# entrpn/learning-jax-sharding

Hardware: AMD Instinct MI355X
Metric: step-time ms + TFLOPS/GPU, case6 sharded attention block at 1/2/4/8 MI355X (higher is better)
Workload: dtype bf16; 1 GPU; model=case6 attention block (M=640, heads=8x64, bf16 compute, f32 params, Adam), global_batch=64, seq_len=256, parallelism=dp1, mode=train, hip_graph=True, graph_segments=1, steps_per_graph=6, warmup_steps_run=67, comm=none, grad_wire=fp32, loss=y.sum(), rules=reference

## Files before the change

learning_jax_sharding_amd/csrc/kernels/gemm.hip:

```cpp
#include "common.h"
#include <stdio.h>
#include <stdlib.h>
#include <type_traits>

namespace {

constexpr int BK = 64;

struct GemmArgs {
  const bf16_t* A;
  const bf16_t* B;
  void* C;
  const void* bias;
  long lda, ldb, ldc;
  long sA, sB, sC, sBias;
  int M, N, K;
  int batch, splitk, kt_per_split;
  float alpha;
  int flags;
  float* psum;
  const void* res;
  long ldr, sR;
  const bf16_t* bptr[4];
  unsigned long long* trace;
};

constexpr int kTraceSlots = 128;

constexpr int kResAdd = 64, kResMask = 128, kResF32 = 256;
constexpr int kSlabs = 512;
constexpr int kMFast = 1024;
constexpr int kBPtrs = 4096;
constexpr int kSlabVst = 8192;

__device__ __forceinline__ void apply_res8(float* v, int flags, const u32x4& rb, const u32x4& rf0,
                                           const u32x4& rf1) {
  float r[8];
  if (flags & kResF32) {
#pragma unroll
    for (int e = 0; e < 4; ++e) { r[e] = __uint_as_float(rf0[e]); r[4 + e] = __uint_as_float(rf1[e]); }
  } else {
#pragma unroll
    for (int e = 0; e < 4; ++e) {
      r[2 * e] = __uint_as_float(rb[e] << 16);
      r[2 * e + 1] = __uint_as_float(rb[e] & 0xffff0000u);
    }
  }
  if (flags & kResAdd) {
#pragma unroll
    for (int e = 0; e < 8; ++e) v[e] = bf2f(f2bf(v[e])) + bf2f(f2bf(r[e]));
  } else if (flags & kResMask) {
#pragma unroll
    for (int e = 0; e < 8; ++e) v[e] = r[e] > 0.f ? v[e] : 0.f;
  }
}

template <int R>
__device__ __forceinline__ int swz_mn(int krow, int c8) {
  int f;
  if constexpr (R >= 128) f = ((krow & 3) | (((krow >> 3) & 1) << 2)) << 2;
  else f = ((((krow >> 1) & 1)) | (((krow >> 3) & 1) << 1)) << 2;
  return c8 ^ f;
}

__device__ __forceinline__ int swz_k(int row, int c16) { return c16 ^ ((row >> 1) & 7); }

template <int R, bool KC>
struct Stage {
  static constexpr int CHUNKS = R * BK * 2 / 16 / 256;
  u32x4 v[CHUNKS];

  __device__ __forceinline__ void load(const bf16_t* __restrict__ base, long ld, int r0, int k0, int R_lim,
                                       int K, int tid) {
#pragma unroll
    for (int i = 0; i < CHUNKS; ++i) {
      int c = tid + 256 * i;
      if constexpr (KC) {
        int row = c >> 3, kc = c & 7;
        int gr = r0 + row, gk = k0 + kc * 8;
        if (gr < R_lim && gk < K)
          v[i] = *reinterpret_cast<const u32x4*>(base + (long)gr * ld + gk);
        else
          v[i] = u32x4{0, 0, 0, 0};
      } else {
        constexpr int CPR = R / 8;
        int krow = c / CPR, mc = c % CPR;
        int gk = k0 + krow, gr = r0 + mc * 8;
        if (gk < K && gr < R_lim)
          v[i] = *reinterpret_cast<const u32x4*>(base + (long)gk * ld + gr);
        else
          v[i] = u32x4{0, 0, 0, 0};
      }
    }
  }

  __device__ __forceinline__ void store(bf16_t* lds, int tid) const {
#pragma unroll
    for (int i = 0; i < CHUNKS; ++i) {
      int c = tid + 256 * i;
      if constexpr (KC) {
        int row = c >> 3, kc = c & 7;
        *reinterpret_cast<u32x4*>(lds + row * BK + swz_k(row, kc) * 8) = v[i];
      } else {
        constexpr int CPR = R / 8;
        int krow = c / CPR, mc = c % CPR;
        *reinterpret_cast<u32x4*>(lds + krow * R + swz_mn<R>(krow, mc * 2) * 4) = v[i];
      }
    }
  }
};

template <int R, bool KC>
__device__ __forceinline__ bf16x8 frag(const bf16_t* lds, int rb, int ks, int lane) {
  if constexpr (KC) {
    int row = rb + (lane & 15);
    int kc = ks * 4 + (lane >> 4);
    u32x4 raw = *reinterpret_cast<const u32x4*>(lds + row * BK + swz_k(row, kc) * 8);
    return __builtin_bit_cast(bf16x8, raw);
  } else {
    int g = lane >> 4, i = lane & 15, q = i >> 2, p = i & 3;
    int kr0 = ks * 32 + 8 * g + q;
    int c8 = (rb >> 2) + p;
    s16x4 lo = lds_read_tr16(lds + kr0 * R + swz_mn<R>(kr0, c8) * 4);
    int kr1 = kr0 + 4;
    s16x4 hi = lds_read_tr16(lds + kr1 * R + swz_mn<R>(kr1, c8) * 4);
    return join_bf16x8(lo, hi);
  }
}

template <int BM, int BN, bool A_KC, bool B_KC, bool OUT_F32>
__global__ __launch_bounds__(256) void gemm_bf16_kernel(GemmArgs p) {
  constexpr int TM = BM / 32, TN = BN / 32;
  constexpr int A_TILE = BM * BK, B_TILE = BN * BK;
  __shared__ __attribute__((aligned(16))) bf16_t smem[2 * (A_TILE + B_TILE)];
#define As(i) (smem + (i) * A_TILE)
#define Bs(i) (smem + 2 * A_TILE + (i) * B_TILE)

  const int tid = threadIdx.x, lane = tid & 63, wave = tid >> 6;
  const int wr = wave >> 1, wc = wave & 1;
  const int ntm = (p.M + BM - 1) / BM, ntn = (p.N + BN - 1) / BN;
  const int tile = xcd_remap(blockIdx.x, gridDim.x);
  const int tm_i = tile / ntn, tn_i = tile % ntn;
  if (tm_i >= ntm) return;
  const int bz = blockIdx.y;
  const int b = bz / p.splitk, split = bz % p.splitk;
  const int m0 = tm_i * BM, n0 = tn_i * BN;

  const bf16_t* Ab = p.A + (long)b * p.sA;
  const bf16_t* Bb = p.B + (long)b * p.sB;

  const int nkt_total = (p.K + BK - 1) / BK;
  const int kt_begin = split * p.kt_per_split;
  const int kt_end = min(nkt_total, kt_begin + p.kt_per_split);

  f32x4 acc[TM][TN];
#pragma unroll
  for (int i = 0; i < TM; ++i)
#pragma unroll
    for (int j = 0; j < TN; ++j) acc[i][j] = f32x4{0.f, 0.f, 0.f, 0.f};

  Stage<BM, A_KC> sa;
  Stage<BN, B_KC> sb;
  if (kt_begin < kt_end) {
    sa.load(Ab, p.lda, m0, kt_begin * BK, p.M, p.K, tid);
    sb.load(Bb, p.ldb, n0, kt_begin * BK, p.N, p.K, tid);
    sa.store(As(0), tid);
    sb.store(Bs(0), tid);
  }
  __syncthreads();

  for (int kt = kt_begin; kt < kt_end; ++kt) {
    const int cur = (kt - kt_begin) & 1;
    const bool more = kt + 1 < kt_end;
    if (more) {
      sa.load(Ab, p.lda, m0, (kt + 1) * BK, p.M, p.K, tid);
      sb.load(Bb, p.ldb, n0, (kt + 1) * BK, p.N, p.K, tid);
    }
#pragma unroll
    for (int ks = 0; ks < BK / 32; ++ks) {
      bf16x8 af[TM], bfr[TN];
#pragma unroll
      for (int i = 0; i < TM; ++i) af[i] = frag<BM, A_KC>(As(cur), wr * (BM / 2) + i * 16, ks, lane);
#pragma unroll
      for (int j = 0; j < TN; ++j) bfr[j] = frag<BN, B_KC>(Bs(cur), wc * (BN / 2) + j * 16, ks, lane);
#pragma unroll
      for (int i = 0; i < TM; ++i)
#pragma unroll
        for (int j = 0; j < TN; ++j) acc[i][j] = mfma16x16x32(af[i], bfr[j], acc[i][j]);
    }
    if (more) {
      sa.store(As(cur ^ 1), tid);
      sb.store(Bs(cur ^ 1), tid);
    }
    __syncthreads();
  }

  const bool relu = p.flags & 1;
  const bool has_bias = (p.flags & 2) && p.splitk == 1;
  const bool bias_f32 = p.flags & 4;
  const bool accumulate = p.flags & 8;
  if constexpr (!OUT_F32) {
    constexpr int LDC = BN + 8;
    bf16_t* ct = smem;
#pragma unroll
    for (int j = 0; j < TN; ++j) {
      const int cl = wc * (BN / 2) + j * 16 + (lane & 15);
      const int col = n0 + cl;
      float bv = 0.f;
      if (has_bias && col < p.N) {
        const long bo = (long)b * p.sBias + col;
        bv = bias_f32 ? reinterpret_cast<const float*>(p.bias)[bo]
                      : bf2f(reinterpret_cast<const bf16_t*>(p.bias)[bo]);
      }
#pragma unroll
      for (int i = 0; i < TM; ++i)
#pragma unroll
        for (int r = 0; r < 4; ++r) {
          float v = acc[i][j][r] * p.alpha + bv;
          if (relu) v = fmaxf(v, 0.f);
          ct[(wr * (BM / 2) + i * 16 + (lane >> 4) * 4 + r) * LDC + cl] = f2bf(v);
        }
    }
    __syncthreads();
    bf16_t* Cb = reinterpret_cast<bf16_t*>(p.C) + (long)b * p.sC;
    constexpr int CPR = BN / 8;
    const bool vec_ok = (p.ldc % 8 == 0) && ((((uintptr_t)Cb) & 15) == 0);
    for (int c = tid; c < BM * CPR; c += 256) {
      const int rl = c / CPR, cc = c % CPR;
      const int row = m0 + rl, col = n0 + cc * 8;
      if (row >= p.M || col >= p.N) continue;
      const bf16_t* src = ct + rl * LDC + cc * 8;
      bf16_t* dst = Cb + (long)row * p.ldc + col;
      if (p.flags & (kResAdd | kResMask)) {
        float v[8];
        u32x4 rb = {0, 0, 0, 0}, rf0 = {0, 0, 0, 0}, rf1 = {0, 0, 0, 0};
        const long ro = (long)b * p.sR + (long)row * p.ldr + col;
#pragma unroll
        for (int e = 0; e < 8; ++e) {
          v[e] = bf2f(src[e]);
          if (col + e < p.N) {
            if (p.flags & kResF32) {
              const float rv = reinterpret_cast<const float*>(p.res)[ro + e];
              if (e < 4) rf0[e] = __float_as_uint(rv); else rf1[e - 4] = __float_as_uint(rv);
            } else {
              const unsigned rv = reinterpret_cast<const bf16_t*>(p.res)[ro + e];
              rb[e >> 1] |= (e & 1) ? (rv << 16) : rv;
            }
          }
        }
        apply_res8(v, p.flags, rb, rf0, rf1);
        if (vec_ok && col + 8 <= p.N)
          *reinterpret_cast<u32x4*>(dst) = u32x4{pack_bf16x2(v[0], v[1]), pack_bf16x2(v[2], v[3]),
                                                 pack_bf16x2(v[4], v[5]), pack_bf16x2(v[6], v[7])};
        else
          for (int e = 0; e < 8 && col + e < p.N; ++e) dst[e] = f2bf(v[e]);
      } else if (vec_ok && col + 8 <= p.N) {
        *reinterpret_cast<u32x4*>(dst) = *reinterpret_cast<const u32x4*>(src);
      } else {
        for (int e = 0; e < 8 && col + e < p.N; ++e) dst[e] = src[e];
      }
    }
    return;
  }
#pragma unroll
  for (int i = 0; i < TM; ++i) {
#pragma unroll
    for (int j = 0; j < TN; ++j) {
      const int col = n0 + wc * (BN / 2) + j * 16 + (lane & 15);
      if (col >= p.N) continue;
      float bv = 0.f;
      if (has_bias) {
        const long bo = (long)b * p.sBias + col;
        bv = bias_f32 ? reinterpret_cast<const float*>(p.bias)[bo]
                      : bf2f(reinterpret_cast<const bf16_t*>(p.bias)[bo]);
      }
#pragma unroll
      for (int r = 0; r < 4; ++r) {
        const int row = m0 + wr * (BM / 2) + i * 16 + (lane >> 4) * 4 + r;
        if (row >= p.M) continue;
        float v = acc[i][j][r] * p.alpha + bv;
        if (relu) v = fmaxf(v, 0.f);
        const long off = (long)b * p.sC + (long)row * p.ldc + col;
        if constexpr (OUT_F32) {
          float* C = reinterpret_cast<float*>(p.C);
          if (p.splitk > 1) atomicAdd(C + off, v);
          else if (accumulate) C[off] += v;
          else C[off] = v;
        } else {
          reinterpret_cast<bf16_t*>(p.C)[off] = f2bf(v);
        }
      }
    }
  }
}

#undef As
#undef Bs


template <int R>
__device__ __forceinline__ int swz_mn16(int krow) {
  if constexpr (R >= 128) return ((krow & 3) | (((krow >> 3) & 1) << 2)) << 1;
  else return ((((krow >> 1) & 1)) | (((krow >> 3) & 1) << 1)) << 1;
}


template <int N>
__device__ __forceinline__ void wait_vm_imm() {
  asm volatile("s_waitcnt vmcnt(%0)" ::"n"(N) : "memory");
}
__device__ __forceinline__ void wait_vm_n(int n) {
  switch (n) {
#define LJS_W(k) case k: wait_vm_imm<k>(); return;
    LJS_W(0) LJS_W(1) LJS_W(2) LJS_W(3) LJS_W(4) LJS_W(5) LJS_W(6) LJS_W(7) LJS_W(8) LJS_W(9) LJS_W(10)
    LJS_W(11) LJS_W(12) LJS_W(13) LJS_W(14) LJS_W(15) LJS_W(16) LJS_W(17) LJS_W(18) LJS_W(19) LJS_W(20)
    LJS_W(21) LJS_W(22) LJS_W(23) LJS_W(24) LJS_W(25) LJS_W(26) LJS_W(27) LJS_W(28) LJS_W(29) LJS_W(30)
    LJS_W(31) LJS_W(32) LJS_W(33) LJS_W(34) LJS_W(35) LJS_W(36) LJS_W(37) LJS_W(38) LJS_W(39) LJS_W(40)
    LJS_W(41) LJS_W(42) LJS_W(43) LJS_W(44) LJS_W(45) LJS_W(46)
#undef LJS_W
    default: wait_vm_imm<47>(); return;
  }
}

template <int R, bool KC, int NW>
struct DmaTile {
  static constexpr int PIECES = R * BK * 2 / 1024;
  static constexpr int PER_WAVE = PIECES / NW;
  static_assert(PIECES % NW == 0, "pieces must split evenly over the waves");
  int voff[PER_WAVE];

  __device__ __forceinline__ void init(long ld, int wave, int lane) {
#pragma unroll
    for (int i = 0; i < PER_WAVE; ++i) {
      const int q = wave + NW * i;
      long e;
      if constexpr (KC) {
        const int row = 8 * q + (lane >> 3), slot = lane & 7;
        e = (long)row * ld + 8 * (slot ^ ((row >> 1) & 7));
      } else {
        constexpr int CPR = R / 8;
        constexpr int KPP = 64 / CPR;
        const int krow = KPP * q + lane / CPR, slot = lane % CPR;
        e = (long)krow * ld + 8 * (slot ^ swz_mn16<R>(krow));
      }
      voff[i] = (int)(e * 2);
    }
  }

  __device__ __forceinline__ void issue(__amdgpu_buffer_rsrc_t rs, bf16_t* lds, int soff, int wave) const {
#pragma unroll
    for (int i = 0; i < PER_WAVE; ++i)
      __builtin_amdgcn_raw_ptr_buffer_load_lds(rs, (LDS_PTR(void))(lds + (wave + NW * i) * 512), 16, voff[i], soff,
                                               0, 0);
  }
};

struct WorkItem {
  int b, m0, n0, kt0, split;
};

__device__ __forceinline__ WorkItem decode_item(const GemmArgs& p, int item, int ntm, int ntn) {
  WorkItem w;
  int tm_i, tn_i, r;
  if (p.flags & kMFast) {
    tm_i = item % ntm;
    r = item / ntm;
    tn_i = r % ntn;
    r /= ntn;
  } else {
    tn_i = item % ntn;
    r = item / ntn;
    tm_i = r % ntm;
    r /= ntm;
  }
  w.b = r % p.batch;
  w.split = r / p.batch;
  w.m0 = tm_i;
  w.n0 = tn_i;
  w.kt0 = w.split * p.kt_per_split;
  return w;
}

constexpr int kSC1 = 16;

template <int BM, int BN, int WM, int WN, int NST, bool A_KC, bool B_KC, bool OUT_F32, int RES = 0>
__device__ __forceinline__ void gemm_dma_body(const GemmArgs& p, const int bid, const int G) {
  constexpr int NW = WM * WN;
  constexpr int TM = BM / WM / 16, TN = BN / WN / 16;
  constexpr int A_TILE = BM * BK, B_TILE = BN * BK, STAGE = A_TILE + B_TILE;
  using TA = DmaTile<BM, A_KC, NW>;
  using TB = DmaTile<BN, B_KC, NW>;
  constexpr int L = TA::PER_WAVE + TB::PER_WAVE;
  constexpr bool SWAP = true;
  static_assert(OUT_F32 || TN % 2 == 0, "column blocks pair up for 16-byte stores");
  constexpr int S_EPI = TM * TN / 2;
  static_assert(L * (NST - 1) + S_EPI + 1 <= 63, "vmcnt immediate range");
  __shared__ __attribute__((aligned(16))) bf16_t smem[NST * STAGE];

  const int tid = threadIdx.x, lane = tid & 63;
  const int wave = __builtin_amdgcn_readfirstlane(tid >> 6);
  const int wr = wave / WN, wc = wave % WN;
  const int ntm = (p.M + BM - 1) / BM, ntn = (p.N + BN - 1) / BN;
  const int items = p.batch * p.splitk * ntm * ntn;
  const int slot = xcd_remap(bid, G);
  const int my_items = slot < items ? (items - slot + G - 1) / G : 0;
  const int nk = p.kt_per_split;
  const int total = my_items * nk;
#ifdef LJS_GEMM_TRACE
  unsigned long long* trc = p.trace ? p.trace + ((long)bid * NW + wave) * kTraceSlots : nullptr;
  int trn = 0;
  auto stamp = [&]() {
    if (trc && trn < kTraceSlots - 1) {
      const unsigned long long t = __builtin_amdgcn_s_memtime();
      if (lane == 0) trc[trn] = t;
    }
    ++trn;
  };
  auto stamp_end = [&]() {
    if (trc) {
      const unsigned long long t = __builtin_amdgcn_s_memtime();
      if (lane == 0) trc[kTraceSlots - 1] = t;
    }
  };
#else
  auto stamp = [&]() {};
  auto stamp_end = [&]() {};
#endif
  stamp();

  constexpr int AES = 2;
  const long a_bytes = AES * (A_KC ? (long)(p.M - 1) * p.lda + p.K : (long)(p.K - 1) * p.lda + p.M);
  const long b_bytes = 2 * (B_KC ? (long)(p.N - 1) * p.ldb + p.K : (long)(p.K - 1) * p.ldb + p.N);
  const long a_kt = A_KC ? (long)BK * AES : (long)BK * p.lda * 2;
  const long b_kt = B_KC ? (long)BK * 2 : (long)BK * p.ldb * 2;

  TA ta;
  TB tb;
  ta.init(p.lda, wave, lane);
  tb.init(p.ldb, wave, lane);

  int is_item = 0, is_kt = 0;
  __amdgpu_buffer_rsrc_t ra, rb;
  int a_off = 0, b_off = 0;
  const int a_step = (int)a_kt, b_step = (int)b_kt;
  auto load_item = [&](int k) {
    const WorkItem w = decode_item(p, slot + G * k, ntm, ntn);
    ra = make_rsrc(reinterpret_cast<const unsigned char*>(p.A) + (long)w.b * p.sA * AES, a_bytes);
    rb = make_rsrc((p.flags & kBPtrs) ? p.bptr[w.b] : p.B + (long)w.b * p.sB, b_bytes);
    a_off = __builtin_amdgcn_readfirstlane(
        (int)((A_KC ? (long)w.m0 * BM * p.lda : (long)w.m0 * BM) * AES + w.kt0 * a_kt));
    b_off = __builtin_amdgcn_readfirstlane(
        (int)((B_KC ? (long)w.n0 * BN * p.ldb : (long)w.n0 * BN) * 2 + w.kt0 * b_kt));
  };
  auto issue_a = [&](int st) { ta.issue(ra, smem + st * STAGE, a_off, wave); };
  auto issue_b = [&](int st) { tb.issue(rb, smem + st * STAGE + A_TILE, b_off, wave); };
  auto issue_next = [&](int st) {
    if (is_kt == 0) load_item(is_item);
    issue_a(st);
    issue_b(st);
    a_off += a_step;
    b_off += b_step;
    if (++is_kt == nk) { is_kt = 0; ++is_item; }
  };
  auto issue_half = [&](int st, bool second) {
    if (!second) {
      if (is_kt == 0) load_item(is_item);
      issue_a(st);
      a_off += a_step;
    } else {
      issue_b(st);
      b_off += b_step;
      if (++is_kt == nk) { is_kt = 0; ++is_item; }
    }
  };

  f32x4 acc[TM][TN];
#pragma unroll
  for (int i = 0; i < TM; ++i)
#pragma unroll
    for (int j = 0; j < TN; ++j) acc[i][j] = f32x4{0.f, 0.f, 0.f, 0.f};

#pragma unroll
  for (int s = 0; s < NST - 1; ++s)
    if (s < total) issue_next(s);

  constexpr bool PLAIN = RES == 3, BSUM = RES == 4, NOALPHA = PLAIN || BSUM;
  constexpr bool HAS_R = RES == 1 || RES == 2;
  const bool relu = !PLAIN && !BSUM && (p.flags & 1);
  const bool has_bias = BSUM || (!PLAIN && (p.flags & 2) && p.splitk == 1);
  const bool bias_f32 = BSUM || (p.flags & 4);
  const bool accumulate = !PLAIN && (p.flags & 8);
  const bool st_sc1 = p.flags & 32;
  const bool psum_on = !OUT_F32 && !PLAIN && p.psum != nullptr;
  float tsum = 0.f;
  const bool slabs = OUT_F32 && (PLAIN || (p.flags & kSlabs));
  const __amdgpu_buffer_rsrc_t rc = make_rsrc(
      p.C, (OUT_F32 ? 4 : 2) *
               ((long)((slabs ? p.splitk * p.batch : p.batch) - 1) * p.sC + (long)(p.M - 1) * p.ldc + p.N));
  bool after_epi = false;

  auto wait_landed = [&](int g) {
    stamp();
    const bool tail = g + NST - 2 >= total;
    if constexpr (NST >= 3) {
      if (tail) asm volatile("s_waitcnt vmcnt(0)" ::: "memory");
      else if (SWAP && after_epi && psum_on)
        asm volatile("s_waitcnt vmcnt(%0)" ::"n"(L * (NST - 2) + S_EPI + 1) : "memory");
      else if (SWAP && after_epi) asm volatile("s_waitcnt vmcnt(%0)" ::"n"(L * (NST - 2) + S_EPI) : "memory");
      else asm volatile("s_waitcnt vmcnt(%0)" ::"n"(L * (NST - 2)) : "memory");
    } else {
      if (SWAP && after_epi && psum_on) asm volatile("s_waitcnt vmcnt(%0)" ::"n"(S_EPI + 1) : "memory");
      else if (SWAP && after_epi) asm volatile("s_waitcnt vmcnt(%0)" ::"n"(S_EPI) : "memory");
      else asm volatile("s_waitcnt vmcnt(0)" ::: "memory");
    }
    after_epi = false;
    stamp();
    asm volatile("s_waitcnt lgkmcnt(0)" ::: "memory");
    __builtin_amdgcn_s_barrier();
    stamp();
  };
  bf16x8 ka[TM], kb[TN], la[TM], lb[TN];
  auto read_frags = [&](int g, int ks, bf16x8* af, bf16x8* bfr) {
    const bf16_t* As_ = smem + (g % NST) * STAGE;
    const bf16_t* Bs_ = As_ + A_TILE;
#pragma unroll
    for (int ii = 0; ii < TM; ++ii) af[ii] = frag<BM, A_KC>(As_, wr * (BM / WM) + ii * 16, ks, lane);
#pragma unroll
    for (int j = 0; j < TN; ++j) bfr[j] = frag<BN, B_KC>(Bs_, wc * (BN / WN) + j * 16, ks, lane);
  };
  auto mfmas = [&](const bf16x8* af, const bf16x8* bfr) {
#pragma unroll
    for (int ii = 0; ii < TM; ++ii)
#pragma unroll
      for (int j = 0; j < TN; ++j) {
        if constexpr (SWAP) acc[ii][j] = mfma16x16x32(bfr[j], af[ii], acc[ii][j]);
        else acc[ii][j] = mfma16x16x32(af[ii], bfr[j], acc[ii][j]);
      }
  };
  static_assert(BK == 64, "two k-steps per K-tile");
#ifndef LJS_GEMM_PIN
#define LJS_GEMM_PIN 0
#endif
  auto pin = [&](bf16x8* af, bf16x8* bfr) {
#if LJS_GEMM_PIN
    __builtin_amdgcn_sched_barrier(0);
#pragma unroll
    for (int ii = 0; ii < TM; ++ii) asm volatile("" : "+v"(af[ii]));
#pragma unroll
    for (int j = 0; j < TN; ++j) asm volatile("" : "+v"(bfr[j]));
#endif
  };
  constexpr bool ONE_PER_CU = !(NW == 4 && NST * (BM + BN) * 64 * 2 <= 80 * 1024);
  constexpr bool PIPE = (TM + TN <= 8 || (NW == 8 && TM + TN <= 10) || (NW == 4 && ONE_PER_CU && TM + TN <= 16)) &&
                        A_KC && B_KC;
  if (PIPE && total > 0) {
    wait_landed(0);
    read_frags(0, 0, ka, kb);
    if (NST - 1 < total) issue_next((NST - 1) % NST);
  }

  for (int it = 0, f = 0; it < my_items; ++it) {
  for (int kk = 0; kk < nk; ++kk, ++f) {
    if constexpr (!PIPE) {
      wait_landed(f);
      const bool more = f + NST - 1 < total;
      const int nst = (f + NST - 1) % NST;
      read_frags(f, 0, ka, kb);
      if (more) issue_half(nst, false);
      mfmas(ka, kb);
      read_frags(f, 1, la, lb);
      if (more) issue_half(nst, true);
      mfmas(la, lb);
      continue;
    }
    read_frags(f, 1, la, lb);
    mfmas(ka, kb);
    pin(la, lb);
    const bool inner = kk + 1 < nk;
    const bool more = inner && f + NST < total;
    if (inner) {
      wait_landed(f + 1);
      read_frags(f + 1, 0, ka, kb);
      if (more) issue_half(f % NST, false);
    }
    mfmas(la, lb);
    if (more) issue_half(f % NST, true);
  }

    const WorkItem w = decode_item(p, slot + G * it, ntm, ntn);
    const int m0 = w.m0 * BM + wr * (BM / WM), n0 = w.n0 * BN + wc * (BN / WN);
    const int g = lane >> 4;
    if constexpr (!OUT_F32) {
      const bool even = (g & 1) == 0;
      u32x4 rv[2][TN / 2][RES == 2 ? 2 : 1];
      __amdgpu_buffer_rsrc_t rr;
      if constexpr (HAS_R)
        rr = make_rsrc(p.res, (RES == 2 ? 4 : 2) * ((long)(p.batch - 1) * p.sR + (long)(p.M - 1) * p.ldr + p.N));
      auto load_r = [&](int ii) {
        if constexpr (HAS_R) {
#pragma unroll
          for (int q = 0; q < TN / 2; ++q) {
            const int col = n0 + 16 * (even ? 2 * q : 2 * q + 1) + 4 * (g & ~1);
            const int row = m0 + ii * 16 + (lane & 15);
            const bool ok = row < p.M && col < p.N;
            const int off = ok ? (int)(((long)w.b * p.sR + (long)row * p.ldr + col) * (RES == 2 ? 4 : 2)) : 0x7ffffff0;
            rv[ii & 1][q][0] = __builtin_amdgcn_raw_buffer_load_b128(rr, off, 0, 0);
            if constexpr (RES == 2)
              rv[ii & 1][q][RES == 2 ? 1 : 0] = __builtin_amdgcn_raw_buffer_load_b128(rr, ok ? off + 16 : off, 0, 0);
          }
        }
      };
      load_r(0);
      float bvs[TN / 2][8];
      const bool bias_vec = has_bias && ((((uintptr_t)p.bias) & 15) == 0) && (p.sBias % 8) == 0;
#pragma unroll
      for (int q = 0; q < TN / 2; ++q) {
        const int col = n0 + 16 * (even ? 2 * q : 2 * q + 1) + 4 * (g & ~1);
        const long bo = (long)w.b * p.sBias + col;
        if (bias_vec && col + 8 <= p.N) {
          if (bias_f32) {
            const f32x4 lo = *reinterpret_cast<const f32x4*>(reinterpret_cast<const float*>(p.bias) + bo);
            const f32x4 hi = *reinterpret_cast<const f32x4*>(reinterpret_cast<const float*>(p.bias) + bo + 4);
#pragma unroll
            for (int e = 0; e < 4; ++e) {
              bvs[q][e] = lo[e];
              bvs[q][4 + e] = hi[e];
            }
          } else {
            const u32x4 u = *reinterpret_cast<const u32x4*>(reinterpret_cast<const bf16_t*>(p.bias) + bo);
#pragma unroll
            for (int e = 0; e < 4; ++e) {
              bvs[q][2 * e] = __uint_as_float(u[e] << 16);
              bvs[q][2 * e + 1] = __uint_as_float(u[e] & 0xffff0000u);
            }
          }
          continue;
        }
#pragma unroll
        for (int e = 0; e < 8; ++e) {
          bvs[q][e] = 0.f;
          if (has_bias && col + e < p.N) {
            bvs[q][e] = bias_f32 ? reinterpret_cast<const float*>(p.bias)[bo + e]
                                 : bf2f(reinterpret_cast<const bf16_t*>(p.bias)[bo + e]);
          }
        }
      }
#pragma unroll
      for (int ii = 0; ii < TM; ++ii) {
        if (ii + 1 < TM) load_r(ii + 1);
#pragma unroll
        for (int q = 0; q < TN / 2; ++q) {
          const int col = n0 + 16 * (even ? 2 * q : 2 * q + 1) + 4 * (g & ~1);
          const float* bv = bvs[q];
          const f32x4 a0 = NOALPHA ? acc[ii][2 * q] : acc[ii][2 * q] * p.alpha;
          const f32x4 a1 = NOALPHA ? acc[ii][2 * q + 1] : acc[ii][2 * q + 1] * p.alpha;
          acc[ii][2 * q] = f32x4{0.f, 0.f, 0.f, 0.f};
          acc[ii][2 * q + 1] = f32x4{0.f, 0.f, 0.f, 0.f};
          float v[8];
          pair_rows16(a0, a1, even, v);
          u32x4 pk;
          if constexpr (!PLAIN) {
#pragma unroll
            for (int e = 0; e < 8; ++e) {
              v[e] += bv[e];
              if (relu) v[e] = fmaxf(v[e], 0.f);
            }
          }
          if constexpr (HAS_R) apply_res8(v, p.flags, rv[ii & 1][q][0], rv[ii & 1][q][0], rv[ii & 1][q][RES == 2 ? 1 : 0]);
#pragma unroll
          for (int e = 0; e < 4; ++e) pk[e] = pack_bf16x2(v[2 * e], v[2 * e + 1]);
          const int row = m0 + ii * 16 + (lane & 15);
          const bool ok = row < p.M && col < p.N;
          const int off = ok ? (int)(((long)w.b * p.sC + (long)row * p.ldc + col) * 2) : 0x7ffffff0;
          if (st_sc1) __builtin_amdgcn_raw_buffer_store_b128(pk, rc, off, 0, kSC1);
          else __builtin_amdgcn_raw_buffer_store_b128(pk, rc, off, 0, 0);
          if (psum_on && ok) {
#pragma unroll
            for (int e = 0; e < 4; ++e) tsum += __uint_as_float(pk[e] << 16) + __uint_as_float(pk[e] & 0xffff0000u);
          }
        }
      }
      if (psum_on) {
        tsum = warp_sum64(tsum);
        if (lane == 0) p.psum[(long)(slot + G * it) * NW + wave] = tsum;
        tsum = 0.f;
      }
      after_epi = true;
    } else {
      const bool vec = (p.ldc & 3) == 0 && (p.sC & 3) == 0 && ((((uintptr_t)p.C) & 15) == 0);
      if constexpr (BN / WN == 64 && WM * WN * (BM / WM) * 256 <= NST * STAGE * 2) {
        if (slabs && vec && (p.flags & kSlabVst) && it + 1 == my_items && !has_bias && !relu && !accumulate) {
          __syncthreads();
          unsigned char* img = reinterpret_cast<unsigned char*>(smem) + wave * (BM / WM) * 256;
#pragma unroll
          for (int ii = 0; ii < TM; ++ii) {
            const int r = ii * 16 + (lane & 15);
#pragma unroll
            for (int j = 0; j < TN; ++j)
              *reinterpret_cast<f32x4*>(img + r * 256 + (((4 * j + g) ^ (r & 7)) << 4)) = PLAIN ? acc[ii][j] : acc[ii][j] * p.alpha;
          }
          asm volatile("s_waitcnt lgkmcnt(0)" ::: "memory");
          const long cb = (long)(w.split * p.batch + w.b) * p.sC;
#pragma unroll
          for (int q = 0; q < (BM / WM) / 4; ++q) {
            const int r = 4 * q + (lane >> 4), c = lane & 15;
            const f32x4 v = *reinterpret_cast<const f32x4*>(img + r * 256 + ((c ^ (r & 7)) << 4));
            const int row = m0 + r, col = n0 + 4 * c;
            if (row < p.M && col + 4 <= p.N) {
              const u32x4 bits = __builtin_bit_cast(u32x4, v);
              __builtin_amdgcn_raw_buffer_store_b128(bits, rc, (int)((cb + (long)row * p.ldc + col) * 4), 0, 0);
            } else if (row < p.M) {
              float* C = reinterpret_cast<float*>(p.C) + cb + (long)row * p.ldc + col;
#pragma unroll
              for (int e = 0; e < 4; ++e)
                if (col + e < p.N) C[e] = v[e];
            }
          }
          continue;
        }
      }
      const long cb = (long)(slabs ? w.split * p.batch + w.b : w.b) * p.sC;
#pragma unroll
      for (int j = 0; j < TN; ++j) {
        const int col = n0 + j * 16 + 4 * g;
        float bv[4] = {0.f, 0.f, 0.f, 0.f};
        if (has_bias) {
#pragma unroll
          for (int e = 0; e < 4; ++e) {
            if (col + e >= p.N) continue;
            const long bo = (long)w.b * p.sBias + col + e;
            bv[e] = bias_f32 ? reinterpret_cast<const float*>(p.bias)[bo]
                             : bf2f(reinterpret_cast<const bf16_t*>(p.bias)[bo]);
          }
        }
#pragma unroll
        for (int ii = 0; ii < TM; ++ii) {
          const int row = m0 + ii * 16 + (lane & 15);
          f32x4 v;
#pragma unroll
          for (int e = 0; e < 4; ++e) {
            v[e] = PLAIN ? acc[ii][j][e] : acc[ii][j][e] * p.alpha + bv[e];
            if (relu) v[e] = fmaxf(v[e], 0.f);
          }
          acc[ii][j] = f32x4{0.f, 0.f, 0.f, 0.f};
          if (row >= p.M || col >= p.N) continue;
          float* C = reinterpret_cast<float*>(p.C) + cb + (long)row * p.ldc + col;
          if (p.splitk > 1 && !slabs) {
#pragma unroll
            for (int e = 0; e < 4; ++e)
              if (col + e < p.N) atomicAdd(C + e, v[e]);
          } else if (vec && col + 4 <= p.N) {
            if (accumulate) v += *reinterpret_cast<const f32x4*>(C);
            const int off = (int)((cb + (long)row * p.ldc + col) * 4);
            const u32x4 bits = __builtin_bit_cast(u32x4, v);
            if (st_sc1) __builtin_amdgcn_raw_buffer_store_b128(bits, rc, off, 0, kSC1);
            else __builtin_amdgcn_raw_buffer_store_b128(bits, rc, off, 0, 0);
          } else {
#pragma unroll
            for (int e = 0; e < 4; ++e)
              if (col + e < p.N) C[e] = accumulate ? C[e] + v[e] : v[e];
          }
        }
      }
      if (it + 1 < my_items) asm volatile("s_waitcnt vmcnt(0)" ::: "memory");
    }
    if (PIPE && f < total) {
      wait_landed(f);
      read_frags(f, 0, ka, kb);
      if (f + NST - 1 < total) issue_next((f + NST - 1) % NST);
    }
  }
  stamp_end();
}

template <int BM, int BN, int WM, int WN, int NST, bool A_KC, bool B_KC, bool OUT_F32, int RES = 0>
__global__ __launch_bounds__(WM * WN * 64, (WM * WN == 4 && NST * (BM + BN) * 64 * 2 <= 80 * 1024) ? 2 : 1) void
gemm_dma_kernel(GemmArgs p) {
  gemm_dma_body<BM, BN, WM, WN, NST, A_KC, B_KC, OUT_F32, RES>(p, blockIdx.x, gridDim.x);
}

template <int BM, int BN, int WM, int WN, int NST, bool A_KC, bool B_KC, bool OUT_F32, int RES = 0>
__global__ __launch_bounds__(WM * WN * 64, (WM * WN == 4 && NST * (BM + BN) * 64 * 2 <= 80 * 1024) ? 2 : 1) void
gemm_dma_group2_kernel(GemmArgs p0, GemmArgs p1, int g0) {
  if ((int)blockIdx.x < g0)
    gemm_dma_body<BM, BN, WM, WN, NST, A_KC, B_KC, OUT_F32, RES>(p0, blockIdx.x, g0);
  else
    gemm_dma_body<BM, BN, WM, WN, NST, A_KC, B_KC, OUT_F32, RES>(p1, blockIdx.x - g0, gridDim.x - g0);
}

template <int BM, int BN, int WM, int WN, int NST, int RES>
__global__ __launch_bounds__(WM * WN * 64, (WM * WN == 4 && NST * (BM + BN) * 64 * 2 <= 80 * 1024) ? 2 : 1) void
gemm_lean_kernel(GemmArgs p) {
  constexpr int NW = WM * WN;
  constexpr int TM = BM / WM / 16, TN = BN / WN / 16;
  constexpr int A_TILE = BM * BK, B_TILE = BN * BK, STAGE = A_TILE + B_TILE;
  using TA = DmaTile<BM, true, NW>;
  using TB = DmaTile<BN, true, NW>;
  constexpr int L = TA::PER_WAVE + TB::PER_WAVE;
  static_assert(TN % 2 == 0, "column blocks pair up for 16-byte stores");
  static_assert(NST >= 2, "at least one K-tile in flight");
  constexpr int S_EPI = TM * TN / 2;
  static_assert(L * (NST - 1) + S_EPI + 1 <= 63, "vmcnt immediate range");
  constexpr bool PLAIN = RES == 3, BSUM = RES == 4, NOALPHA = PLAIN || BSUM;
  constexpr bool HAS_R = RES == 1 || RES == 2;
  __shared__ __attribute__((aligned(16))) bf16_t smem[NST * STAGE];

  const int tid = threadIdx.x, lane = tid & 63;
  const int wave = __builtin_amdgcn_readfirstlane(tid >> 6);
  const int wr = wave / WN, wc = wave % WN;
  const int ntm = (p.M + BM - 1) / BM, ntn = (p.N + BN - 1) / BN;
  const int items = p.batch * ntm * ntn;
  const int G = gridDim.x;
  const int slot = xcd_remap(blockIdx.x, G);
  const int my_items = slot < items ? (items - slot + G - 1) / G : 0;
  if (my_items == 0) return;
  const int nk = p.kt_per_split;

  const long a_bytes = 2 * ((long)(p.M - 1) * p.lda + p.K);
  const long b_bytes = 2 * ((long)(p.N - 1) * p.ldb + p.K);
  TA ta;
  TB tb;
  ta.init(p.lda, wave, lane);
  tb.init(p.ldb, wave, lane);

  int is_item = 0, is_kt = 0;
  __amdgpu_buffer_rsrc_t ra, rb;
  int a_off = 0, b_off = 0;
  auto load_item = [&](int k) {
    const WorkItem w = decode_item(p, slot + G * (k < my_items ? k : 0), ntm, ntn);
    ra = make_rsrc(p.A + (long)w.b * p.sA, a_bytes);
    rb = make_rsrc(p.B + (long)w.b * p.sB, b_bytes);
    a_off = __builtin_amdgcn_readfirstlane((int)((long)w.m0 * BM * p.lda * 2));
    b_off = __builtin_amdgcn_readfirstlane((int)((long)w.n0 * BN * p.ldb * 2));
    if (k >= my_items) {
      ra = make_rsrc(p.A, 0);
      rb = make_rsrc(p.B, 0);
    }
  };
  auto issue_a = [&](int so) { ta.issue(ra, smem + so, a_off, wave); };
  auto issue_b = [&](int so) { tb.issue(rb, smem + so + A_TILE, b_off, wave); };
  auto advance = [&]() {
    a_off += BK * 2;
    b_off += BK * 2;
    if (++is_kt == nk) {
      is_kt = 0;
      load_item(++is_item);
    }
  };

  f32x4 acc[TM][TN];
#pragma unroll
  for (int i = 0; i < TM; ++i)
#pragma unroll
    for (int j = 0; j < TN; ++j) acc[i][j] = f32x4{0.f, 0.f, 0.f, 0.f};

  load_item(0);
#pragma unroll
  for (int s = 0; s < NST - 1; ++s) {
    issue_a(s * STAGE);
    issue_b(s * STAGE);
    advance();
  }

  const bool relu = !PLAIN && !BSUM && (p.flags & 1);
  const bool has_bias = BSUM || (!PLAIN && (p.flags & 2));
  const bool bias_f32 = BSUM || (p.flags & 4);
  const bool st_sc1 = p.flags & 32;
  const bool psum_on = !PLAIN && p.psum != nullptr;
  const __amdgpu_buffer_rsrc_t rc = make_rsrc(p.C, 2 * ((long)(p.batch - 1) * p.sC + (long)(p.M - 1) * p.ldc + p.N));

  bf16x8 ka[TM], kb[TN], la[TM], lb[TN];
  auto read_frags = [&](int so, int ks, bf16x8* af, bf16x8* bfr) {
    const bf16_t* As_ = smem + so;
    const bf16_t* Bs_ = As_ + A_TILE;
#pragma unroll
    for (int ii = 0; ii < TM; ++ii) af[ii] = frag<BM, true>(As_, wr * (BM / WM) + ii * 16, ks, lane);
#pragma unroll
    for (int j = 0; j < TN; ++j) bfr[j] = frag<BN, true>(Bs_, wc * (BN / WN) + j * 16, ks, lane);
  };
  auto mfmas = [&](const bf16x8* af, const bf16x8* bfr) {
#pragma unroll
    for (int ii = 0; ii < TM; ++ii)
#pragma unroll
      for (int j = 0; j < TN; ++j) acc[ii][j] = mfma16x16x32(bfr[j], af[ii], acc[ii][j]);
  };
  auto next_so = [](int so) { return so + STAGE == NST * STAGE ? 0 : so + STAGE; };
  auto barrier = []() {
    asm volatile("s_waitcnt lgkmcnt(0)" ::: "memory");
    __builtin_amdgcn_s_barrier();
  };

  int so = (NST - 1) * STAGE;
  auto item_start = [&](bool after_epi) {
    if (!after_epi) asm volatile("s_waitcnt vmcnt(%0)" ::"n"(L * (NST - 2)) : "memory");
    else if (psum_on) asm volatile("s_waitcnt vmcnt(%0)" ::"n"(L * (NST - 2) + S_EPI + 1) : "memory");
    else asm volatile("s_waitcnt vmcnt(%0)" ::"n"(L * (NST - 2) + S_EPI) : "memory");
    barrier();
    const int nso = next_so(so);
    read_frags(nso, 0, ka, kb);
    issue_a(so);
    issue_b(so);
    advance();
    so = nso;
  };
  item_start(false);

  float tsum = 0.f;
  for (int it = 0; it < my_items; ++it) {
    for (int kk = 0; kk + 1 < nk; ++kk) {
      read_frags(so, 1, la, lb);
      mfmas(ka, kb);
      const int nso = next_so(so);
      asm volatile("s_waitcnt vmcnt(%0)" ::"n"(L * (NST - 2)) : "memory");
      barrier();
      read_frags(nso, 0, ka, kb);
      issue_a(so);
      mfmas(la, lb);
      issue_b(so);
      advance();
      so = nso;
    }
    read_frags(so, 1, la, lb);
    mfmas(ka, kb);
    mfmas(la, lb);

    const WorkItem w = decode_item(p, slot + G * it, ntm, ntn);
    const int m0 = w.m0 * BM + wr * (BM / WM), n0 = w.n0 * BN + wc * (BN / WN);
    const int g = lane >> 4;
    const bool even = (g & 1) == 0;
    u32x4 rv[2][TN / 2][RES == 2 ? 2 : 1];
    __amdgpu_buffer_rsrc_t rr;
    if constexpr (HAS_R)
      rr = make_rsrc(p.res, (RES == 2 ? 4 : 2) * ((long)(p.batch - 1) * p.sR + (long)(p.M - 1) * p.ldr + p.N));
    auto load_r = [&](int ii) {
      if constexpr (HAS_R) {
#pragma unroll
        for (int q = 0; q < TN / 2; ++q) {
          const int col = n0 + 16 * (even ? 2 * q : 2 * q + 1) + 4 * (g & ~1);
          const int row = m0 + ii * 16 + (lane & 15);
          const bool ok = row < p.M && col < p.N;
          const int off = ok ? (int)(((long)w.b * p.sR + (long)row * p.ldr + col) * (RES == 2 ? 4 : 2)) : 0x7ffffff0;
          rv[ii & 1][q][0] = __builtin_amdgcn_raw_buffer_load_b128(rr, off, 0, 0);
          if constexpr (RES == 2)
            rv[ii & 1][q][RES == 2 ? 1 : 0] = __builtin_amdgcn_raw_buffer_load_b128(rr, ok ? off + 16 : off, 0, 0);
        }
      }
    };
    load_r(0);
    float bvs[TN / 2][8];
    const bool bias_vec = has_bias && ((((uintptr_t)p.bias) & 15) == 0) && (p.sBias % 8) == 0;
#pragma unroll
    for (int q = 0; q < TN / 2; ++q) {
      const int col = n0 + 16 * (even ? 2 * q : 2 * q + 1) + 4 * (g & ~1);
      const long bo = (long)w.b * p.sBias + col;
      if (bias_vec && col + 8 <= p.N) {
        if (bias_f32) {
          const f32x4 lo = *reinterpret_cast<const f32x4*>(reinterpret_cast<const float*>(p.bias) + bo);
          const f32x4 hi = *reinterpret_cast<const f32x4*>(reinterpret_cast<const float*>(p.bias) + bo + 4);
#pragma unroll
          for (int e = 0; e < 4; ++e) {
            bvs[q][e] = lo[e];
            bvs[q][4 + e] = hi[e];
          }
        } else {
          const u32x4 u = *reinterpret_cast<const u32x4*>(reinterpret_cast<const bf16_t*>(p.bias) + bo);
#pragma unroll
          for (int e = 0; e < 4; ++e) {
            bvs[q][2 * e] = __uint_as_float(u[e] << 16);
            bvs[q][2 * e + 1] = __uint_as_float(u[e] & 0xffff0000u);
          }
        }
        continue;
      }
#pragma unroll
      for (int e = 0; e < 8; ++e) {
        bvs[q][e] = 0.f;
        if (has_bias && col + e < p.N) {
          bvs[q][e] = bias_f32 ? reinterpret_cast<const float*>(p.bias)[bo + e]
                               : bf2f(reinterpret_cast<const bf16_t*>(p.bias)[bo + e]);
        }
      }
    }
#pragma unroll
    for (int ii = 0; ii < TM; ++ii) {
      if (ii + 1 < TM) load_r(ii + 1);
#pragma unroll
      for (int q = 0; q < TN / 2; ++q) {
        const int col = n0 + 16 * (even ? 2 * q : 2 * q + 1) + 4 * (g & ~1);
        const float* bv = bvs[q];
        const f32x4 a0 = NOALPHA ? acc[ii][2 * q] : acc[ii][2 * q] * p.alpha;
        const f32x4 a1 = NOALPHA ? acc[ii][2 * q + 1] : acc[ii][2 * q + 1] * p.alpha;
        acc[ii][2 * q] = f32x4{0.f, 0.f, 0.f, 0.f};
        acc[ii][2 * q + 1] = f32x4{0.f, 0.f, 0.f, 0.f};
        float v[8];
        pair_rows16(a0, a1, even, v);
        u32x4 pk;
        if constexpr (!PLAIN) {
#pragma unroll
          for (int e = 0; e < 8; ++e) {
            v[e] += bv[e];
            if (relu) v[e] = fmaxf(v[e], 0.f);
          }
        }
        if constexpr (HAS_R) apply_res8(v, p.flags, rv[ii & 1][q][0], rv[ii & 1][q][0], rv[ii & 1][q][RES == 2 ? 1 : 0]);
#pragma unroll
        for (int e = 0; e < 4; ++e) pk[e] = pack_bf16x2(v[2 * e], v[2 * e + 1]);
        const int row = m0 + ii * 16 + (lane & 15);
        const bool ok = row < p.M && col < p.N;
        const int off = ok ? (int)(((long)w.b * p.sC + (long)row * p.ldc + col) * 2) : 0x7ffffff0;
        if (st_sc1) __builtin_amdgcn_raw_buffer_store_b128(pk, rc, off, 0, kSC1);
        else __builtin_amdgcn_raw_buffer_store_b128(pk, rc, off, 0, 0);
        if (psum_on && ok) {
#pragma unroll
          for (int e = 0; e < 4; ++e) tsum += __uint_as_float(pk[e] << 16) + __uint_as_float(pk[e] & 0xffff0000u);
        }
      }
    }
    if (psum_on) {
      tsum = warp_sum64(tsum);
      if (lane == 0) p.psum[(long)(slot + G * it) * NW + wave] = tsum;
      tsum = 0.f;
    }
    if (it + 1 < my_items) item_start(true);
  }
  asm volatile("s_waitcnt vmcnt(0)" ::: "memory");
}


#define LJS_DMA_INST(BM, BN, WM, WN, NST, AK, BKc, OF) \
  template __global__ void gemm_dma_kernel<BM, BN, WM, WN, NST, AK, BKc, OF>(GemmArgs);
#define LJS_DMA_INST_LAYOUTS(NST)                                                                           \
  LJS_DMA_INST(128, 128, 2, 2, NST, true, true, false) LJS_DMA_INST(128, 128, 2, 2, NST, true, true, true)     \
  LJS_DMA_INST(128, 128, 2, 2, NST, false, false, false) LJS_DMA_INST(128, 128, 2, 2, NST, false, false, true) \
  LJS_DMA_INST(128, 128, 2, 2, NST, true, false, false) LJS_DMA_INST(128, 128, 2, 2, NST, true, false, true)   \
  LJS_DMA_INST(128, 128, 2, 2, NST, false, true, false) LJS_DMA_INST(128, 128, 2, 2, NST, false, true, true)
LJS_DMA_INST_LAYOUTS(2)
LJS_DMA_INST_LAYOUTS(4)
template __global__ void gemm_dma_kernel<128, 128, 2, 2, 2, false, false, true, 3>(GemmArgs);
template __global__ void gemm_dma_group2_kernel<128, 128, 2, 2, 2, false, false, true, 3>(GemmArgs, GemmArgs, int);
template __global__ void gemm_dma_group2_kernel<128, 128, 2, 4, 4, false, false, true, 3>(GemmArgs, GemmArgs, int);
template __global__ void gemm_dma_group2_kernel<128, 128, 2, 4, 3, false, false, true, 3>(GemmArgs, GemmArgs, int);
template __global__ void gemm_dma_kernel<128, 128, 2, 4, 4, false, false, true, 3>(GemmArgs);
template __global__ void gemm_dma_kernel<128, 128, 2, 4, 3, false, false, true, 3>(GemmArgs);
#define LJS_DMA_INST_64(NST)                                                                               \
  LJS_DMA_INST(64, 64, 2, 2, NST, true, true, false) LJS_DMA_INST(64, 64, 2, 2, NST, true, true, true)     \
  LJS_DMA_INST(64, 64, 2, 2, NST, false, false, false) LJS_DMA_INST(64, 64, 2, 2, NST, false, false, true) \
  LJS_DMA_INST(64, 64, 2, 2, NST, true, false, false) LJS_DMA_INST(64, 64, 2, 2, NST, true, false, true)   \
  LJS_DMA_INST(64, 64, 2, 2, NST, false, true, false) LJS_DMA_INST(64, 64, 2, 2, NST, false, true, true)
LJS_DMA_INST_64(3)
LJS_DMA_INST_64(4)
#undef LJS_DMA_INST_64
LJS_DMA_INST(256, 128, 4, 2, 3, true, true, false)
LJS_DMA_INST(256, 128, 4, 2, 3, true, true, true)
LJS_DMA_INST(256, 192, 4, 2, 2, true, true, false)
LJS_DMA_INST(256, 128, 4, 2, 3, false, false, true)
LJS_DMA_INST(128, 256, 2, 4, 3, false, false, true)
LJS_DMA_INST(128, 160, 4, 1, 2, true, true, false)
#define LJS_DMA_INST_8W(NST)                                                                                \
  LJS_DMA_INST(128, 128, 2, 4, NST, false, false, true) LJS_DMA_INST(128, 128, 2, 4, NST, true, true, false) \
  LJS_DMA_INST(128, 128, 2, 4, NST, true, true, true)
LJS_DMA_INST_8W(3)
LJS_DMA_INST_8W(4)
#undef LJS_DMA_INST_8W
#define LJS_DMA_INST_RES(BM, BN, WM, WN, NST) \
  template __global__ void gemm_dma_kernel<BM, BN, WM, WN, NST, true, true, false, 1>(GemmArgs); \
  template __global__ void gemm_dma_kernel<BM, BN, WM, WN, NST, true, true, false, 2>(GemmArgs); \
  template __global__ void gemm_dma_kernel<BM, BN, WM, WN, NST, true, true, false, 3>(GemmArgs); \
// ... 478 lines not shown
```

Measured before the change: 702.0 TFLOPS, whole job (matmul FLOPs of fwd+bwd summed over the n_gpus GPUs; the per-GPU rate the metric names is tflops_per_gpu = value / n_gpus).

## Add half-stage LDS ring pipeline with hand-scheduled transpose reads for weight-grad GEMM

For the 128x128, two-stage, MN-major, f32 plain-output GEMM variant, the LDS buffering is replaced by a five-slot ring of half-k-tiles. Each iteration issues the next half-tile loads while computing, and the transposed LDS reads are issued in grouped inline asm with explicit lgkmcnt waits so MFMAs on the first fragment row can start early. The epilogue now always uses 16-byte buffer stores, with out-of-range offsets standing in for bounds checks. Vmcnt accounting is adjusted so epilogue stores are not fully drained before the next item. The aim is better load/compute overlap and fewer stalls, at the cost of complex hand-tuned counters that are fragile to correctness and scheduling errors.

```diff
diff --git a/learning_jax_sharding_amd/csrc/kernels/gemm.hip b/learning_jax_sharding_amd/csrc/kernels/gemm.hip
--- a/learning_jax_sharding_amd/csrc/kernels/gemm.hip
+++ b/learning_jax_sharding_amd/csrc/kernels/gemm.hip
@@ -24,6 +24,39 @@
   const bf16_t* bptr[4];
   unsigned long long* trace;
 };
+
+#define LJS_TR2(l, h, a) "ds_read_b64_tr_b16 %" #l ", %" #a "\n\tds_read_b64_tr_b16 %" #h ", %" #a " offset:1024\n\t"
+__device__ __forceinline__ void tr_read5_wait(s16x4* lo, s16x4* hi, const unsigned* ad) {
+  asm volatile(LJS_TR2(0, 1, 10) LJS_TR2(2, 3, 11) LJS_TR2(4, 5, 12) LJS_TR2(6, 7, 13) LJS_TR2(8, 9, 14)
+               "s_waitcnt lgkmcnt(0)"
+               : "=&v"(lo[0]), "=&v"(hi[0]), "=&v"(lo[1]), "=&v"(hi[1]), "=&v"(lo[2]), "=&v"(hi[2]), "=&v"(lo[3]),
+                 "=&v"(hi[3]), "=&v"(lo[4]), "=&v"(hi[4])
+               : "v"(ad[0]), "v"(ad[1]), "v"(ad[2]), "v"(ad[3]), "v"(ad[4])
+               : "memory");
+}
+__device__ __forceinline__ void tr_read3(s16x4* lo, s16x4* hi, const unsigned* ad) {
+  asm volatile(LJS_TR2(0, 1, 6) LJS_TR2(2, 3, 7) LJS_TR2(4, 5, 8)
+               : "=&v"(lo[0]), "=&v"(hi[0]), "=&v"(lo[1]), "=&v"(hi[1]), "=&v"(lo[2]), "=&v"(hi[2])
+               : "v"(ad[0]), "v"(ad[1]), "v"(ad[2])
+               : "memory");
+}
+__device__ __forceinline__ void tr_read4(s16x4* lo, s16x4* hi, const unsigned* ad) {
+  asm volatile(LJS_TR2(0, 1, 8) LJS_TR2(2, 3, 9) LJS_TR2(4, 5, 10) LJS_TR2(6, 7, 11)
+               : "=&v"(lo[0]), "=&v"(hi[0]), "=&v"(lo[1]), "=&v"(hi[1]), "=&v"(lo[2]), "=&v"(hi[2]), "=&v"(lo[3]),
+                 "=&v"(hi[3])
+               : "v"(ad[0]), "v"(ad[1]), "v"(ad[2]), "v"(ad[3])
+               : "memory");
+}
+#undef LJS_TR2
+#define LJS_TRW(x, i) "+v"(x##lo[i]), "+v"(x##hi[i])
+__device__ __forceinline__ void tr_wait3_8(s16x4* alo, s16x4* ahi, s16x4* blo, s16x4* bhi) {
+  asm volatile("s_waitcnt lgkmcnt(0)"
+               : LJS_TRW(a, 0), LJS_TRW(a, 1), LJS_TRW(a, 2), LJS_TRW(b, 0), LJS_TRW(b, 1), LJS_TRW(b, 2),
+                 LJS_TRW(b, 3), LJS_TRW(b, 4), LJS_TRW(b, 5), LJS_TRW(b, 6), LJS_TRW(b, 7)
+               :
+               : "memory");
+}
+#undef LJS_TRW
 
 constexpr int kTraceSlots = 128;
 
@@ -126,6 +159,13 @@
     s16x4 hi = lds_read_tr16(lds + kr1 * R + swz_mn<R>(kr1, c8) * 4);
     return join_bf16x8(lo, hi);
   }
+}
+
+__device__ __forceinline__ unsigned frag_tr_addr(const bf16_t* lds, int rb, int lane) {
+  const int g = lane >> 4, i = lane & 15, q = i >> 2, p = i & 3;
+  const int kr0 = 8 * g + q;
+  const int c8 = (rb >> 2) + p;
+  return (unsigned)(unsigned long)(LDS_PTR(const bf16_t))(lds + kr0 * 128 + swz_mn<128>(kr0, c8) * 4);
 }
 
 template <int BM, int BN, bool A_KC, bool B_KC, bool OUT_F32>
@@ -353,6 +393,15 @@
       __builtin_amdgcn_raw_ptr_buffer_load_lds(rs, (LDS_PTR(void))(lds + (wave + NW * i) * 512), 16, voff[i], soff,
                                                0, 0);
   }
+
+  template <int H>
+  __device__ __forceinline__ void issue_half(__amdgpu_buffer_rsrc_t rs, bf16_t* lds, int soff, int wave) const {
+    static_assert(!KC && PER_WAVE == 4 && R == 128, "pieces i and i + 2 are 32 k-rows apart");
+#pragma unroll
+    for (int i = 0; i < 2; ++i)
+      __builtin_amdgcn_raw_ptr_buffer_load_lds(rs, (LDS_PTR(void))(lds + (wave + NW * i) * 512), 16, voff[2 * H + i],
+                                               soff, 0, 0);
+  }
 };
 
 struct WorkItem {
@@ -395,7 +444,11 @@
   static_assert(OUT_F32 || TN % 2 == 0, "column blocks pair up for 16-byte stores");
   constexpr int S_EPI = TM * TN / 2;
   static_assert(L * (NST - 1) + S_EPI + 1 <= 63, "vmcnt immediate range");
-  __shared__ __attribute__((aligned(16))) bf16_t smem[NST * STAGE];
+  constexpr bool RING = NST == 2 && BM == 128 && BN == 128 && NW == 4 && !A_KC && !B_KC && OUT_F32 && RES == 3;
+  constexpr int HALF = STAGE / 2, A_HALF = A_TILE / 2, RING_SLOTS = 5;
+  constexpr int E_RING = TM * TN;
+  static_assert(!RING || 4 * L / 2 + E_RING + 1 <= 63, "vmcnt immediate range");
+  __shared__ __attribute__((aligned(16))) bf16_t smem[RING ? RING_SLOTS * HALF : NST * STAGE];
 
   const int tid = threadIdx.x, lane = tid & 63;
   const int wave = __builtin_amdgcn_readfirstlane(tid >> 6);
@@ -422,9 +475,15 @@
       if (lane == 0) trc[kTraceSlots - 1] = t;
     }
   };
+  auto stamp_st = [&]() {
+    const int st = trc && trn < kTraceSlots - 1;
+    stamp();
+    return st;
+  };
 #else
   auto stamp = [&]() {};
   auto stamp_end = [&]() {};
+  auto stamp_st = [&]() { return 0; };
 #endif
   stamp();
 
@@ -480,9 +539,39 @@
 #pragma unroll
     for (int j = 0; j < TN; ++j) acc[i][j] = f32x4{0.f, 0.f, 0.f, 0.f};
 
-#pragma unroll
-  for (int s = 0; s < NST - 1; ++s)
-    if (s < total) issue_next(s);
+  int ring_w = 0, ring_r = 0;
+  auto ring_adv = [](int so, int n) {
+    so += n * HALF;
+    return so >= RING_SLOTS * HALF ? so - RING_SLOTS * HALF : so;
+  };
+  auto ring_issue0 = [&]() {
+    if constexpr (RING) {
+      if (is_kt == 0) load_item(is_item);
+      ta.template issue_half<0>(ra, smem + ring_w, a_off, wave);
+      tb.template issue_half<0>(rb, smem + ring_w + A_HALF, b_off, wave);
+      ring_w = ring_adv(ring_w, 1);
+    }
+  };
+  auto ring_issue1 = [&]() {
+    if constexpr (RING) {
+      ta.template issue_half<1>(ra, smem + ring_w, a_off, wave);
+      tb.template issue_half<1>(rb, smem + ring_w + A_HALF, b_off, wave);
+      ring_w = ring_adv(ring_w, 1);
+      a_off += a_step;
+      b_off += b_step;
+      if (++is_kt == nk) { is_kt = 0; ++is_item; }
+    }
+  };
+
+  if constexpr (RING) {
+    if (total > 0) { ring_issue0(); ring_issue1(); }
+    if (total > 1) { ring_issue0(); ring_issue1(); }
+    if (total > 2) ring_issue0();
+  } else {
+#pragma unroll
+    for (int s = 0; s < NST - 1; ++s)
+      if (s < total) issue_next(s);
+  }
 
   constexpr bool PLAIN = RES == 3, BSUM = RES == 4, NOALPHA = PLAIN || BSUM;
   constexpr bool HAS_R = RES == 1 || RES == 2;
@@ -519,6 +608,22 @@
     __builtin_amdgcn_s_barrier();
     stamp();
   };
+  int ring_epi = 0;
+  auto ring_wait = [&](int f) {
+    const int st = stamp_st();
+    const int n = f == 0 ? (total > 2 ? 3 : 2 * total - 2) : (f + 1 < total ? 1 : 0);
+    if (n == 1 && !ring_epi) {
+      if (st) asm volatile("s_waitcnt vmcnt(5)" ::: "memory");
+      else asm volatile("s_waitcnt vmcnt(4)" ::: "memory");
+    } else {
+      wait_vm_n(4 * n + ring_epi + st);
+    }
+    ring_epi = 0;
+    stamp();
+    asm volatile("s_waitcnt lgkmcnt(0)" ::: "memory");
+    __builtin_amdgcn_s_barrier();
+    stamp();
+  };
   bf16x8 ka[TM], kb[TN], la[TM], lb[TN];
   auto read_frags = [&](int g, int ks, bf16x8* af, bf16x8* bfr) {
     const bf16_t* As_ = smem + (g % NST) * STAGE;
@@ -561,6 +666,49 @@
 
   for (int it = 0, f = 0; it < my_items; ++it) {
   for (int kk = 0; kk < nk; ++kk, ++f) {
+    if constexpr (RING) {
+      const bf16_t* h0 = smem + ring_r;
+      const bf16_t* h1 = smem + ring_adv(ring_r, 1);
+      ring_r = ring_adv(ring_r, 2);
+      auto addr_half = [&](const bf16_t* hs, unsigned* ad) {
+        ad[0] = frag_tr_addr(hs, wr * (BM / WM), lane);
+#pragma unroll
+        for (int j = 0; j < TN; ++j) ad[1 + j] = frag_tr_addr(hs + A_HALF, wc * (BN / WN) + j * 16, lane);
+#pragma unroll
+        for (int ii = 1; ii < TM; ++ii) ad[4 + ii] = frag_tr_addr(hs, wr * (BM / WM) + ii * 16, lane);
+      };
+      auto row0 = [&](const s16x4* lo, const s16x4* hi) {
+        const bf16x8 a0 = join_bf16x8(lo[0], hi[0]);
+#pragma unroll
+        for (int j = 0; j < TN; ++j) acc[0][j] = mfma16x16x32(join_bf16x8(lo[1 + j], hi[1 + j]), a0, acc[0][j]);
+      };
+      auto rows123 = [&](const s16x4* lo, const s16x4* hi) {
+#pragma unroll
+        for (int ii = 1; ii < TM; ++ii) {
+          const bf16x8 a = join_bf16x8(lo[4 + ii], hi[4 + ii]);
+#pragma unroll
+          for (int j = 0; j < TN; ++j) acc[ii][j] = mfma16x16x32(join_bf16x8(lo[1 + j], hi[1 + j]), a, acc[ii][j]);
+        }
+      };
+      static_assert(TM == 4 && TN == 4 && SWAP, "the tr_read* groups are written for 4 x 4 fragments");
+      unsigned ad0[8], ad1[8];
+      s16x4 r0lo[8], r0hi[8], r1lo[8], r1hi[8];
+      addr_half(h0, ad0);
+      addr_half(h1, ad1);
+      ring_wait(f);
+      tr_read5_wait(r0lo, r0hi, ad0);
+      tr_read3(r0lo + 5, r0hi + 5, ad0 + 5);
+      tr_read4(r1lo, r1hi, ad1);
+      tr_read4(r1lo + 4, r1hi + 4, ad1 + 4);
+      if (f >= 1 && f + 1 < total) ring_issue1();
+      if (f >= 1 && f + 2 < total) ring_issue0();
+      row0(r0lo, r0hi);
+      tr_wait3_8(r0lo + 5, r0hi + 5, r1lo, r1hi);
+      rows123(r0lo, r0hi);
+      row0(r1lo, r1hi);
+      rows123(r1lo, r1hi);
+      continue;
+    }
     if constexpr (!PIPE) {
       wait_landed(f);
       const bool more = f + NST - 1 < total;
@@ -688,6 +836,7 @@
       after_epi = true;
     } else {
       const bool vec = (p.ldc & 3) == 0 && (p.sC & 3) == 0 && ((((uintptr_t)p.C) & 15) == 0);
+      [[maybe_unused]] const bool ring_exact = RING && vec && (p.N & 3) == 0;
       if constexpr (BN / WN == 64 && WM * WN * (BM / WM) * 256 <= NST * STAGE * 2) {
         if (slabs && vec && (p.flags & kSlabVst) && it + 1 == my_items && !has_bias && !relu && !accumulate) {
           __syncthreads();
@@ -743,6 +892,16 @@
             if (relu) v[e] = fmaxf(v[e], 0.f);
           }
           acc[ii][j] = f32x4{0.f, 0.f, 0.f, 0.f};
+          if constexpr (RING) {
+            if (ring_exact) {
+              const bool ok = row < p.M && col < p.N;
+              const int off = ok ? (int)((cb + (long)row * p.ldc + col) * 4) : 0x7ffffff0;
+              const u32x4 bits = __builtin_bit_cast(u32x4, v);
+              if (st_sc1) __builtin_amdgcn_raw_buffer_store_b128(bits, rc, off, 0, kSC1);
+              else __builtin_amdgcn_raw_buffer_store_b128(bits, rc, off, 0, 0);
+              continue;
+            }
+          }
           if (row >= p.M || col >= p.N) continue;
           float* C = reinterpret_cast<float*>(p.C) + cb + (long)row * p.ldc + col;
           if (p.splitk > 1 && !slabs) {
@@ -762,7 +921,8 @@
           }
         }
       }
-      if (it + 1 < my_items) asm volatile("s_waitcnt vmcnt(0)" ::: "memory");
+      if constexpr (RING) ring_epi = ring_exact ? E_RING : 0;
+      else if (it + 1 < my_items) asm volatile("s_waitcnt vmcnt(0)" ::: "memory");
     }
     if (PIPE && f < total) {
       wait_landed(f);
```

Measured after the change: 720.3 TFLOPS, whole job (matmul FLOPs of fwd+bwd summed over the n_gpus GPUs; the per-GPU rate the metric names is tflops_per_gpu = value / n_gpus) (median of 6 runs). 1.03x the previous value.
